# seungjunlee96/lightning-generative-models

Measured on AMD Instinct MI355X. Metric: training images/sec (DDPM UNet 32x32, bs=128), higher is better.
Workload: dtype f32; 1 GPU; configs/diffusion/ddpm.json UNet dim=64, 3x32x32 synthetic NCHW fp32, training_step+backward+Adam+EMA; global_batch=128, per_gpu_batch=128, parallelism=dp1, launch=hipGraph replay (1 graph/step)

## Files before the change

include/lgm_hip.h:

```cpp
#ifndef LGM_HIP_H
#define LGM_HIP_H

#include <stdint.h>

#ifdef __cplusplus
extern "C" {
#endif

#define LGM_ABI_VERSION 7
#define LGM_OK 0
#define LGM_ERR_INVALID (-1)
#define LGM_ERR_UNSUPPORTED (-2)

int lgm_abi_version(void);
const char* lgm_last_error(void);
const char* lgm_last_kernel(void);
int lgm_kernel_name_count(void);
const char* lgm_kernel_name(int i);

typedef struct {
  int32_t B, H, W, Cw;
  int32_t Ho, Wo, Nw;
  int32_t KH, KW, stride, pad;
} LgmConvGeom;
// ... 103 lines not shown
                    const float* g, float* gx, int64_t gx_pitch, int accumulate_gx, const float* res,
                    int64_t res_pitch, float* gg, float gg_beta, int64_t npix, int C, void* workspace, void* stream);
int lgm_rmsnorm_bwd_deferred(const float* x, int64_t x_pitch, const float* gy, int64_t gy_pitch,
                             const float* g, float* gx, int64_t gx_pitch, int accumulate_gx, const float* res,
                             int64_t res_pitch, float* gg, float gg_beta, int64_t npix, int C, void* workspace,
                             int64_t* desc, void* stream);

int lgm_linattn_fwd(const float* qkv, int64_t qkv_pitch, const float* mem_kv, int B, int n,
                    int heads, int dim_head, int M, float* out, int64_t out_pitch, float* ctx,
                    float* kmax, float* ksum, void* stream);
int64_t lgm_rms_qkv_fused_supported(int C, int N);
int lgm_rms_qkv_fused(const float* x, int64_t x_pitch, const float* g, const float* w, int C, int N, int64_t npix,
                      float* xn, int64_t xn_pitch, float* qkv, int64_t qkv_pitch, void* stream);
int64_t lgm_linattn_fwd_fused_supported(int heads, int dim_head, int Cout);
int lgm_linattn_fwd_fused(const float* qkv, int64_t qkv_pitch, const float* mem_kv, int B, int n, int heads,
                          int dim_head, int M, const float* wout, const float* bout, const float* g, int Cout,
                          const float* x, int64_t x_pitch, float* out, int64_t out_pitch, float* o2,
                          int64_t o2_pitch, float* y, int64_t y_pitch, float* ctx, float* kmax, float* ksum,
                          void* stream);
int64_t lgm_linattn_bwd_workspace(int B, int heads, int dim_head, int M);
int lgm_linattn_bwd(const float* qkv, int64_t qkv_pitch, const float* mem_kv, const float* gout,
                    int64_t gout_pitch, const float* ctx, const float* kmax, const float* ksum,
                    int B, int n, int heads, int dim_head, int M, float* gqkv, int64_t gqkv_pitch,
                    float* gmem_kv, float gmem_beta, void* workspace, void* stream);
int64_t lgm_linattn_bwd_fused_supported(int heads, int dim_head, int C);
int64_t lgm_linattn_bwd_fused_slabs(int B, int n, int C);
int64_t lgm_linattn_bwd_fused_workspace(int B, int heads, int dim_head);
int lgm_linattn_bwd_fused(const float* qkv, int64_t qkv_pitch, const float* mem_kv, const float* gout,
                          int64_t gout_pitch, const float* ctx, const float* kmax, const float* ksum,
                          const float* xn, int64_t xn_pitch, const float* wqkv_t, int C, int B, int n,
                          int heads, int dim_head, int M, float* gxn, int64_t gxn_pitch, float* gwqkv,
                          float gw_beta, void* slabs, int64_t slab_bytes, int64_t* gw_desc, float* gmem_kv,
                          float gmem_beta, void* gmem_part, int64_t* gmem_desc, void* workspace, void* stream);
int lgm_linattn_bwd_deferred(const float* qkv, int64_t qkv_pitch, const float* mem_kv, const float* gout,
                             int64_t gout_pitch, const float* ctx, const float* kmax, const float* ksum,
                             int B, int n, int heads, int dim_head, int M, float* gqkv, int64_t gqkv_pitch,
                             float* gmem_kv, float gmem_beta, void* gmem_part, int64_t* gmem_desc,
                             void* workspace, void* stream);
int lgm_attn_bwd_deferred(const float* qkv, int64_t qkv_pitch, const float* mem_kv, const float* out,
                          int64_t out_pitch, const float* gout, int64_t gout_pitch, const float* lse, int B,
                          int n, int heads, int dim_head, int M, float* gqkv, int64_t gqkv_pitch,
                          float* gmem_kv, float gmem_beta, void* gmem_part, int64_t* gmem_desc, void* stream);
int lgm_attn_fwd(const float* qkv, int64_t qkv_pitch, const float* mem_kv, int B, int n, int heads,
                 int dim_head, int M, float* out, int64_t out_pitch, float* lse, void* stream);
int64_t lgm_attn_bwd_workspace(int B, int heads, int dim_head, int M);
int lgm_attn_bwd(const float* qkv, int64_t qkv_pitch, const float* mem_kv, const float* out,
                 int64_t out_pitch, const float* gout, int64_t gout_pitch, const float* lse, int B,
                 int n, int heads, int dim_head, int M, float* gqkv, int64_t gqkv_pitch,
                 float* gmem_kv, float gmem_beta, void* workspace, void* stream);

int lgm_posemb(const int64_t* t, int B, int dim, const float* freqs, float* out, int64_t pitch, void* stream);

#define LGM_ACT_NONE 0
#define LGM_ACT_SILU 1
#define LGM_ACT_GELU 2
#define LGM_ACT_RELU 3
#define LGM_ACT_LRELU 4
#define LGM_ACT_TANH 5
int lgm_act_fwd(const float* x, int64_t x_pitch, const float* bias, const float* res,
                int64_t res_pitch, float* y, int64_t y_pitch, int64_t rows, int cols, int act,
                float slope, void* stream);
int lgm_act_bwd(const float* x, int64_t x_pitch, const float* bias, const float* gy,
                int64_t gy_pitch, float* gx, int64_t gx_pitch, int accumulate, int64_t rows,
                int cols, int act, float slope, void* stream);
int lgm_axpby(const float* a, int64_t a_pitch, float alpha, const float* b, int64_t b_pitch,
              float beta, float* y, int64_t y_pitch, int64_t rows, int cols, void* stream);
// ... 247 lines not shown
```

lightning-generative-models_amd/csrc/attention.hip:

```cpp
#include "lgm_common.h"

int lgm_linattn_ctx_launch(int mode, const float* qkv, long pitch, const float* mem_kv, const float* gout,
                           long gout_pitch, const float* ctx_in, int B, int n, int heads, int M, float scale,
                           float* ctx_out, float* kmax, float* ksum, float* r_out, hipStream_t s,
                           const float* kmax_in = nullptr, const float* ksum_in = nullptr,
                           float* gmem_partial = nullptr);
int lgm_linattn_bwd_fused_launch(const float* qkv, long pitch, const float* gout, long gout_pitch, const float* ctx,
                                 const float* gctx, const float* kmax, const float* ksum, const float* rvec,
                                 const float* xn, long xn_pitch, const float* wt, int B, int n, float scale,
                                 float* gxn, long gxn_pitch, float* slabs, int* blocks_out, hipStream_t s);
int lgm_wgrad_reduce_launch(const float* ws, long slab, float* gw, long n_w, float* gb, long n_b, int splits, float beta,
                            hipStream_t s);
int lgm_linattn_out_fused_launch(const float* qkv, long pitch, const float* ctx, const float* wout, const float* bout,
                                 const float* g, const float* x, long x_pitch, float* ao, long ao_pitch, float* o2,
                                 long o2_pitch, float* y, long y_pitch, int B, int n, int Cout, float scale, hipStream_t s);
int lgm_linattn_bwd_launch(const float* qkv, long pitch, const float* mem_kv, const float* gout, long gout_pitch,
                           const float* ctx, const float* gctx, const float* kmax, const float* ksum,
                           const float* rvec, int B, int n, int heads, int M, float scale, float* gqkv,
                           long gq_pitch, float* gmem_partial, hipStream_t s);
int lgm_attn_tiled_fwd_launch(const float* qkv, long pitch, const float* mem_kv, int B, int n, int heads, int M,
                              float scale, float* out, long out_pitch, float* lse, hipStream_t s);
int lgm_attn_tiled_bwd_launch(const float* qkv, long pitch, const float* mem_kv, const float* out, long out_pitch,
                              const float* gout, long gout_pitch, const float* lse, int B, int n, int heads, int M,
                              float scale, float* gqkv, long gq_pitch, float* gmem_partial, hipStream_t s);

namespace {

constexpr int DH = 32;
constexpr int TI = 64;


__global__ __launch_bounds__(256) void linattn_out_kernel(const float* __restrict__ qkv, long pitch,
                                                          const float* __restrict__ ctx, int n, int heads, float scale,
                                                          float* __restrict__ out, long out_pitch) {
  __shared__ float Qs[TI][DH + 1];
  __shared__ __align__(16) float Cs[DH][DH];
  const int bh = blockIdx.x;
  const int b = bh / heads, h = bh % heads;
  const int i0 = blockIdx.y * TI;
  const int tid = threadIdx.x;
  const int d_l = tid % DH, pl = tid / DH;
  for (int k = tid; k < DH * DH; k += 256) Cs[k / DH][k % DH] = ctx[(long)bh * DH * DH + k];
  {
// ... 488 lines not shown
    gmem_desc[3] = ncols; gmem_desc[4] = 0; gmem_desc[5] = 0; gmem_desc[6] = B; gmem_desc[7] = bb.i;
    return LGM_OK;
  }
  return lgm_wgrad_reduce_launch(part, ncols, gmem_kv, ncols, nullptr, 0, B, gmem_beta, s);
}
}

extern "C" int lgm_linattn_bwd(const float* qkv, int64_t qkv_pitch, const float* mem_kv, const float* gout,
                               int64_t gout_pitch, const float* ctx, const float* kmax, const float* ksum, int B,
                               int n, int heads, int dim_head, int M, float* gqkv, int64_t gqkv_pitch,
                               float* gmem_kv, float gmem_beta, void* workspace, void* stream) {
  LGM_REQUIRE(workspace, "linattn_bwd: null pointer");
  const long bh = (long)B * heads;
  float* part = (float*)workspace + bh * DH * DH + bh * DH;
  return linattn_bwd_impl(qkv, qkv_pitch, mem_kv, gout, gout_pitch, ctx, kmax, ksum, B, n, heads, dim_head, M, gqkv,
                          gqkv_pitch, gmem_kv, gmem_beta, part, nullptr, workspace, stream);
}

extern "C" int lgm_linattn_bwd_deferred(const float* qkv, int64_t qkv_pitch, const float* mem_kv, const float* gout,
                                        int64_t gout_pitch, const float* ctx, const float* kmax, const float* ksum,
                                        int B, int n, int heads, int dim_head, int M, float* gqkv, int64_t gqkv_pitch,
                                        float* gmem_kv, float gmem_beta, void* gmem_part, int64_t* gmem_desc,
                                        void* workspace, void* stream) {
  LGM_REQUIRE(gmem_desc && gmem_part && lgm_aligned16(gmem_kv), "linattn_bwd_deferred: descriptor / partial buffer / aligned gradient required");
  return linattn_bwd_impl(qkv, qkv_pitch, mem_kv, gout, gout_pitch, ctx, kmax, ksum, B, n, heads, dim_head, M, gqkv,
                          gqkv_pitch, gmem_kv, gmem_beta, (float*)gmem_part, gmem_desc, workspace, stream);
}

extern "C" int64_t lgm_linattn_bwd_fused_workspace(int B, int heads, int dim_head) {
  const int64_t bh = (int64_t)B * heads;
  return (bh * dim_head * dim_head + bh * dim_head) * (int64_t)sizeof(float) + 64;
}

extern "C" int lgm_linattn_bwd_fused(const float* qkv, int64_t qkv_pitch, const float* mem_kv, const float* gout,
                                     int64_t gout_pitch, const float* ctx, const float* kmax, const float* ksum,
                                     const float* xn, int64_t xn_pitch, const float* wqkv_t, int C, int B, int n,
                                     int heads, int dim_head, int M, float* gxn, int64_t gxn_pitch, float* gwqkv,
                                     float gw_beta, void* slabs, int64_t slab_bytes, int64_t* gw_desc, float* gmem_kv,
                                     float gmem_beta, void* gmem_part, int64_t* gmem_desc, void* workspace,
                                     void* stream) {
  if (int rc = attn_check(B, n, heads, dim_head, M)) return rc;
  LGM_REQUIRE(lgm_linattn_bwd_fused_supported(heads, dim_head, C), "linattn_bwd_fused: heads=%d dim_head=%d C=%d unsupported",
              heads, dim_head, C);
  LGM_REQUIRE(qkv && mem_kv && gout && ctx && kmax && ksum && xn && wqkv_t && gxn && gwqkv && slabs && gmem_kv && gmem_part &&
                  workspace, "linattn_bwd_fused: null pointer");
  LGM_REQUIRE(qkv_pitch % 4 == 0 && gout_pitch % 4 == 0 && xn_pitch % 4 == 0 && gxn_pitch % 4 == 0 && lgm_aligned16(qkv) &&
                  lgm_aligned16(gout) && lgm_aligned16(ctx) && lgm_aligned16(kmax) && lgm_aligned16(ksum) &&
                  lgm_aligned16(xn) && lgm_aligned16(wqkv_t) && lgm_aligned16(gxn) && lgm_aligned16(gwqkv) &&
                  lgm_aligned16(slabs) && lgm_aligned16(workspace) && lgm_aligned16(gmem_kv) && lgm_aligned16(gmem_part),
              "linattn_bwd_fused: 16-byte aligned operands required");
  LGM_REQUIRE(slab_bytes >= lgm_linattn_bwd_fused_slabs(B, n, C), "linattn_bwd_fused: slab buffer too small");
  hipStream_t s = (hipStream_t)stream;
  const float scale = 1.f / sqrtf((float)dim_head);
  const long bh = (long)B * heads;
  float* gctx = (float*)workspace;
  float* rvec = gctx + bh * DH * DH;
  const long ncols = 2L * heads * DH * M;
  if (int rc = lgm_linattn_ctx_launch(1, qkv, (long)qkv_pitch, mem_kv, gout, (long)gout_pitch, ctx, B, n, heads, M, scale,
                                      gctx, nullptr, nullptr, rvec, s, kmax, ksum, (float*)gmem_part))
    return rc;
  int blocks = 0;
  if (int rc = lgm_linattn_bwd_fused_launch(qkv, (long)qkv_pitch, gout, (long)gout_pitch, ctx, gctx, kmax, ksum, rvec, xn,
                                            (long)xn_pitch, wqkv_t, B, n, scale, gxn, (long)gxn_pitch, (float*)slabs,
                                            &blocks, s))
    return rc;
  union { float f; int64_t i; } bb;
  if (M > 0) {
    if (gmem_desc) {
      bb.i = 0; bb.f = gmem_beta;
      gmem_desc[0] = (int64_t)(uintptr_t)gmem_part; gmem_desc[1] = ncols; gmem_desc[2] = (int64_t)(uintptr_t)gmem_kv;
      gmem_desc[3] = ncols; gmem_desc[4] = 0; gmem_desc[5] = 0; gmem_desc[6] = B; gmem_desc[7] = bb.i;
    } else if (int rc = lgm_wgrad_reduce_launch((const float*)gmem_part, ncols, gmem_kv, ncols, nullptr, 0, B, gmem_beta, s)) {
      return rc;
    }
  } else if (gmem_desc) {
    gmem_desc[6] = 0;
  }
  const long n_w = 3L * heads * DH * C;
  if (gw_desc) {
    bb.i = 0; bb.f = gw_beta;
    gw_desc[0] = (int64_t)(uintptr_t)slabs; gw_desc[1] = n_w; gw_desc[2] = (int64_t)(uintptr_t)gwqkv; gw_desc[3] = n_w;
    gw_desc[4] = 0; gw_desc[5] = 0; gw_desc[6] = blocks; gw_desc[7] = bb.i;
  } else if (int rc = lgm_wgrad_reduce_launch((const float*)slabs, n_w, gwqkv, n_w, nullptr, 0, blocks, gw_beta, s)) {
    return rc;
  }
  return LGM_OK;
}

extern "C" int lgm_attn_fwd(const float* qkv, int64_t qkv_pitch, const float* mem_kv, int B, int n, int heads,
                            int dim_head, int M, float* out, int64_t out_pitch, float* lse, void* stream) {
  if (int rc = attn_check(B, n, heads, dim_head, M)) return rc;
  LGM_REQUIRE(qkv && mem_kv && out && lse, "attn_fwd: null pointer");
  if (attn_tiled(n))
    return lgm_attn_tiled_fwd_launch(qkv, (long)qkv_pitch, mem_kv, B, n, heads, M, 1.f / sqrtf((float)dim_head), out,
                                     (long)out_pitch, lse, (hipStream_t)stream);
  const size_t smem = (size_t)2 * (n + M) * FA_LD * sizeof(float);
  static const bool no_small = getenv("LGM_NO_SMALL_ATTN") != nullptr;
  if (!no_small && n <= SA_MAXN && M <= 16 && qkv_pitch % 4 == 0 && out_pitch % 4 == 0 && lgm_aligned16(qkv) &&
      lgm_aligned16(out) && lgm_aligned16(mem_kv))
  {
    static bool attr = false;
    if (!attr) {
      hipFuncSetAttribute(reinterpret_cast<const void*>(attn_small_fwd_kernel), hipFuncAttributeMaxDynamicSharedMemorySize,
                          (int)(sa_fwd_floats(SA_MAXN, 16) * sizeof(float)));
      attr = true;
    }
    hipLaunchKernelGGL(attn_small_fwd_kernel, dim3(B * heads), dim3(256), sa_fwd_floats(n, M) * sizeof(float),
                       (hipStream_t)stream, qkv, (long)qkv_pitch, mem_kv, n, heads, M, 1.f / sqrtf((float)dim_head), out,
                       (long)out_pitch, lse);
  }
  else
    hipLaunchKernelGGL(attn_fwd_kernel, dim3(B * heads), dim3(128), smem, (hipStream_t)stream, qkv, (long)qkv_pitch,
                       mem_kv, n, heads, M, 1.f / sqrtf((float)dim_head), out, (long)out_pitch, lse);
  LGM_LAUNCH_CHECK();
  return LGM_OK;
}

extern "C" int64_t lgm_attn_bwd_workspace(int B, int heads, int dim_head, int M) {
  const int64_t ncols = 2LL * heads * M * dim_head;
// ... 81 lines not shown
```

lightning-generative-models_amd/csrc/linattn_fused.hip:

```cpp
#include <type_traits>

#include "lgm_common.h"

int lgm_wgrad_reduce_launch(const float* ws, long slab, float* gw, long n_w, float* gb, long n_b, int splits, float beta,
                            hipStream_t s);

namespace {

constexpr int DH = 32;
constexpr int HEADS = 4;
constexpr int HID = HEADS * DH;
constexpr int C = 64;
constexpr int LD = 36;
constexpr int TP = 128;
constexpr int XLD = 80;
constexpr int WLD = 100;

struct FArgs {
  const float* qkv;  long pitch;
  const float* gout; long gout_pitch;
  const float* ctx; const float* gctx; const float* kmax; const float* ksum; const float* rvec;
  const float* xn;   long xn_pitch;
  const float* wt;
  float* gxn;        long gxn_pitch;
  float* slabs;
  int n, tiles, items, per;
  float scale;
};

__device__ __forceinline__ void load16(const float* p, float (&v)[16]) {
#pragma unroll
  for (int q = 0; q < 4; ++q) {
    const f32x4 t = *reinterpret_cast<const f32x4*>(p + 4 * q);
    v[4 * q] = t[0]; v[4 * q + 1] = t[1]; v[4 * q + 2] = t[2]; v[4 * q + 3] = t[3];
  }
}

__global__ __launch_bounds__(256, 1) void linattn_bwd_fused_kernel(const FArgs p) {
  extern __shared__ __align__(16) float sm[];
  float* Qs = sm;
  float* Ks = Qs + TP * LD;
  float* Vs = Ks + TP * LD;
  float* Gs = Vs + TP * LD;
  float* Cs = Gs + TP * LD;
  float* GCs = Cs + DH * LD;
  float* GCt = GCs + DH * LD;
  float* rr = GCt + DH * LD;
  float* Ws = rr + DH;
  float* Xs = Ws + C * WLD;
  const int tid = threadIdx.x;
  const int lane = tid & 63, wid = tid >> 6;
  const int lr = lane & 31, lh = lane >> 5;
  const int l16 = lane & 15, lq = lane >> 4;
  const int c4 = (tid & 7) * 4, prow = tid >> 3;
  const int srow = 32 * wid + (lane >> 1), spart = (lane & 1) * 16;
  const int it0 = blockIdx.x * p.per, it1 = min(p.items, it0 + p.per);
  if (it0 >= it1) return;

  int w_src[6], w_dst[6];
#pragma unroll
  for (int u = 0; u < 6; ++u) {
    const int e = tid + 256 * u;
    const int c = e / 24, rem = e - 24 * c;
    const int part = rem >> 3, j = rem & 7;
    w_src[u] = c * (3 * HID) + part * HID + 4 * j;
    w_dst[u] = c * WLD + part * DH + 4 * j;
  }

  f32x4 q4[4], k4[4], v4[4], g4[4], km4, ks4, cx4, gc4, w4[6];
  float rr1 = 0.f;
  auto issue = [&](int it, int h) {
    const int b = it / p.tiles, i0 = (it % p.tiles) * TP;
    const int rows = min(TP, p.n - i0);
    const long bh = (long)b * HEADS + h;
#pragma unroll
    for (int u = 0; u < 4; ++u) {
      const int r = prow + 32 * u;
      const long row = (long)b * p.n + i0 + (r < rows ? r : 0);
      const float* qp = p.qkv + row * p.pitch + h * DH + c4;
      q4[u] = *reinterpret_cast<const f32x4*>(qp);
      k4[u] = *reinterpret_cast<const f32x4*>(qp + HID);
      v4[u] = *reinterpret_cast<const f32x4*>(qp + 2 * HID);
      g4[u] = *reinterpret_cast<const f32x4*>(p.gout + row * p.gout_pitch + h * DH + c4);
    }
    km4 = *reinterpret_cast<const f32x4*>(p.kmax + bh * DH + c4);
    ks4 = *reinterpret_cast<const f32x4*>(p.ksum + bh * DH + c4);
    cx4 = *reinterpret_cast<const f32x4*>(p.ctx + bh * DH * DH + tid * 4);
    gc4 = *reinterpret_cast<const f32x4*>(p.gctx + bh * DH * DH + tid * 4);
    if (tid < DH) rr1 = p.rvec[bh * DH + tid];
#pragma unroll
    for (int u = 0; u < 6; ++u) w4[u] = *reinterpret_cast<const f32x4*>(p.wt + w_src[u] + h * DH);
  };

  f32x4 dacc[HEADS][6];
#pragma unroll
  for (int h = 0; h < HEADS; ++h)
#pragma unroll
    for (int t = 0; t < 6; ++t) dacc[h][t] = f32x4{0.f, 0.f, 0.f, 0.f};
  const f32x4 zero4 = {0.f, 0.f, 0.f, 0.f};

  issue(it0, 0);
  for (int it = it0; it < it1; ++it) {
    const int b = it / p.tiles, i0 = (it % p.tiles) * TP;
    const int rows = min(TP, p.n - i0);
    f32x16 acc[2];
#pragma unroll
    for (int a = 0; a < 2; ++a)
#pragma unroll
      for (int r = 0; r < 16; ++r) acc[a][r] = 0.f;
    {
#pragma unroll
      for (int u = 0; u < 4; ++u) {
        const int r = prow + 32 * u;
        const long row = (long)b * p.n + i0 + (r < rows ? r : 0);
#pragma unroll
        for (int hf = 0; hf < 2; ++hf) {
          f32x4 xv = *reinterpret_cast<const f32x4*>(p.xn + row * p.xn_pitch + hf * 32 + c4);
          if (r >= rows) xv = zero4;
          *reinterpret_cast<f32x4*>(Xs + r * XLD + hf * 32 + c4) = xv;
        }
      }
    }
    auto head = [&](auto hc) {
      constexpr int h = decltype(hc)::value;
#pragma unroll
      for (int u = 0; u < 4; ++u) {
        const int r = prow + 32 * u;
        const bool live = r < rows;
        f32x4 kv;
#pragma unroll
        for (int k = 0; k < 4; ++k) kv[k] = __expf(k4[u][k] - km4[k]) * (1.f / ks4[k]);
        *reinterpret_cast<f32x4*>(Qs + r * LD + c4) = live ? q4[u] : zero4;
        *reinterpret_cast<f32x4*>(Ks + r * LD + c4) = live ? kv : zero4;
        *reinterpret_cast<f32x4*>(Vs + r * LD + c4) = live ? v4[u] : zero4;
        *reinterpret_cast<f32x4*>(Gs + r * LD + c4) = live ? g4[u] : zero4;
      }
      {
        const int d = tid >> 3, e0 = (tid & 7) * 4;
// ... 70 lines not shown
        dot += __shfl_xor(dot, 1, 64);
#pragma unroll
        for (int q = 0; q < 4; ++q) {
          f32x4 oq, ok;
#pragma unroll
          for (int k = 0; k < 4; ++k) {
            oq[k] = sv[4 * q + k] * (g1[4 * q + k] - dot);
            ok[k] = kk[4 * q + k] * (t2[4 * q + k] - rv[4 * q + k]);
          }
          *reinterpret_cast<f32x4*>(Qs + srow * LD + spart + 4 * q) = oq;
          *reinterpret_cast<f32x4*>(Ks + srow * LD + spart + 4 * q) = ok;
        }
      }
      lgm_wave_lds_sync();
      {
        float* vp = Vs + (32 * wid + lr) * LD + 4 * lh;
#pragma unroll
        for (int g = 0; g < 4; ++g)
          *reinterpret_cast<f32x4*>(vp + 8 * g) = f32x4{a3[4 * g], a3[4 * g + 1], a3[4 * g + 2], a3[4 * g + 3]};
      }
      lgm_wave_lds_sync();
#pragma unroll
      for (int part = 0; part < 3; ++part) {
        float xb[16], w0[16], w1[16];
        load16((part == 0 ? Qs : part == 1 ? Ks : Vs) + (32 * wid + lr) * LD + 16 * lh, xb);
        load16(Ws + lr * WLD + part * DH + 16 * lh, w0);
        load16(Ws + (32 + lr) * WLD + part * DH + 16 * lh, w1);
#pragma unroll
        for (int s = 0; s < 16; ++s) {
          acc[0] = __builtin_amdgcn_mfma_f32_32x32x2f32(w0[s], xb[s], acc[0], 0, 0, 0);
          acc[1] = __builtin_amdgcn_mfma_f32_32x32x2f32(w1[s], xb[s], acc[1], 0, 0, 0);
        }
      }
      __syncthreads();
      {
        const float* xb = Xs + lq * XLD + 16 * wid + l16;
#pragma unroll 4
        for (int s = 0; s < TP / 4; ++s) {
          const float bv = xb[4 * s * XLD];
#pragma unroll
          for (int part = 0; part < 3; ++part) {
            const float* X = (part == 0 ? Qs : part == 1 ? Ks : Vs) + (4 * s + lq) * LD + l16;
            dacc[h][2 * part] = __builtin_amdgcn_mfma_f32_16x16x4f32(X[0], bv, dacc[h][2 * part], 0, 0, 0);
            dacc[h][2 * part + 1] = __builtin_amdgcn_mfma_f32_16x16x4f32(X[16], bv, dacc[h][2 * part + 1], 0, 0, 0);
          }
        }
        __syncthreads();
      }
    };
    head(std::integral_constant<int, 0>{});
    head(std::integral_constant<int, 1>{});
    head(std::integral_constant<int, 2>{});
    head(std::integral_constant<int, 3>{});
    if (32 * wid + lr < rows) {
      float* o = p.gxn + ((long)b * p.n + i0 + 32 * wid + lr) * p.gxn_pitch + 4 * lh;
#pragma unroll
      for (int a = 0; a < 2; ++a)
#pragma unroll
        for (int g = 0; g < 4; ++g)
          *reinterpret_cast<f32x4*>(o + 32 * a + 8 * g) = f32x4{acc[a][4 * g], acc[a][4 * g + 1], acc[a][4 * g + 2], acc[a][4 * g + 3]};
    }
  }
  {
    float* sl = p.slabs + (long)blockIdx.x * (3 * HID * C);
#pragma unroll
    for (int h = 0; h < HEADS; ++h)
#pragma unroll
      for (int t = 0; t < 6; ++t)
#pragma unroll
        for (int r = 0; r < 4; ++r) {
          const int wrow = (t >> 1) * HID + h * DH + (t & 1) * 16 + 4 * lq + r;
          sl[(long)wrow * C + 16 * wid + l16] = dacc[h][t][r];
        }
  }
}

constexpr size_t kSmem = ((size_t)4 * TP * LD + 3 * DH * LD + DH + C * WLD + TP * XLD) * sizeof(float);

int plan_blocks(int B, int n, int* tiles, int* items, int* per) {
  *tiles = lgm_cdiv(n, TP);
  *items = B * *tiles;
  const int nb = *items < 256 ? *items : 256;
  *per = lgm_cdiv(*items, nb);
  return lgm_cdiv(*items, *per);
}

}

extern "C" int64_t lgm_linattn_bwd_fused_supported(int heads, int dim_head, int Cin) {
  return heads == HEADS && dim_head == DH && Cin == C ? 1 : 0;
}

extern "C" int64_t lgm_linattn_bwd_fused_slabs(int B, int n, int Cin) {
  if (Cin != C) return 0;
  int tiles, items, per;
  const int blocks = plan_blocks(B, n, &tiles, &items, &per);
  return (int64_t)blocks * 3 * HID * C * (int64_t)sizeof(float);
}

int lgm_linattn_bwd_fused_launch(const float* qkv, long pitch, const float* gout, long gout_pitch, const float* ctx,
                                 const float* gctx, const float* kmax, const float* ksum, const float* rvec,
                                 const float* xn, long xn_pitch, const float* wt, int B, int n, float scale,
                                 float* gxn, long gxn_pitch, float* slabs, int* blocks_out, hipStream_t s) {
  FArgs a;
  a.qkv = qkv; a.pitch = pitch; a.gout = gout; a.gout_pitch = gout_pitch;
  a.ctx = ctx; a.gctx = gctx; a.kmax = kmax; a.ksum = ksum; a.rvec = rvec;
  a.xn = xn; a.xn_pitch = xn_pitch; a.wt = wt; a.gxn = gxn; a.gxn_pitch = gxn_pitch;
  a.slabs = slabs; a.n = n; a.scale = scale;
  const int blocks = plan_blocks(B, n, &a.tiles, &a.items, &a.per);
  *blocks_out = blocks;
  lgm_note_kernel(LGM_KNAME("linattn_bwd_fused_kernel"));
  static bool attr = false;
  if (!attr) {
    (void)hipFuncSetAttribute(reinterpret_cast<const void*>(linattn_bwd_fused_kernel),
                              hipFuncAttributeMaxDynamicSharedMemorySize, (int)kSmem);
    attr = true;
  }
  hipLaunchKernelGGL(linattn_bwd_fused_kernel, dim3(blocks), dim3(256), kSmem, s, a);
  LGM_LAUNCH_CHECK();
  return LGM_OK;
}

namespace {

constexpr int OTP = 128;
constexpr int ALD = 132;

struct OArgs {
  const float* qkv;  long pitch;
  const float* ctx;
  const float* wout; const float* bout; const float* g;
  const float* x;    long x_pitch;
  float* ao;         long ao_pitch;
  float* o2;         long o2_pitch;
  float* y;          long y_pitch;
  int n, tiles, items, per;
  float scale;
};

template <int NC>
__global__ __launch_bounds__(256, NC == 2 ? 3 : 1) void linattn_out_fused_kernel(const OArgs p) {
  constexpr int CO = 32 * NC;
  extern __shared__ __align__(16) float sm[];
  float* Ws = sm;
  float* Ct = Ws + CO * ALD;
  const int tid = threadIdx.x;
  const int lane = tid & 63, wid = tid >> 6;
  const int lr = lane & 31, lh = lane >> 5;
  const int it0 = blockIdx.x * p.per, it1 = min(p.items, it0 + p.per);
  if (it0 >= it1) return;
  const float sqrtc = sqrtf((float)CO);
// ... 311 lines not shown
```

lightning-generative-models_amd/lgm_hip/ops.py:

```python
from __future__ import annotations

import ctypes
from typing import Optional

import torch

from ._lib import ConvGeom, lib

ACT_NONE, ACT_SILU, ACT_GELU, ACT_RELU, ACT_LRELU, ACT_TANH = 0, 1, 2, 3, 4, 5


def stream() -> int:
    return torch.cuda.current_stream().cuda_stream


def _p(t: Optional[torch.Tensor]) -> Optional[int]:
    return None if t is None else t.data_ptr()


def pitch(t: torch.Tensor) -> int:
    assert t.stride(-1) == 1 or t.shape[-1] == 1, "last dim must be dense"
    if t.dim() == 1:
        return t.shape[0]
    pt = t.stride(-2)
# ... 962 lines not shown
    L = lib()
    B, H, W, _ = qkv.shape
    ws = workspace(L.lgm_linattn_bwd_workspace(B, heads, dim_head, M), qkv.device)
    if defer is None or gmem_ptr % 16 or M <= 0:
        L.lgm_linattn_bwd(qkv.data_ptr(), pitch(qkv), mem_ptr, gout.data_ptr(), pitch(gout), ctx.data_ptr(),
                          kstat[0].data_ptr(), kstat[1].data_ptr(), B, H * W, heads, dim_head, M, gqkv.data_ptr(),
                          pitch(gqkv), gmem_ptr, gmem_beta, ws.data_ptr(), stream())
        return
    nb = B * 2 * heads * dim_head * M * 4
    part = _persistent((gmem_ptr, nb), nb, qkv.device)
    desc = (ctypes.c_int64 * 8)()
    L.lgm_linattn_bwd_deferred(qkv.data_ptr(), pitch(qkv), mem_ptr, gout.data_ptr(), pitch(gout), ctx.data_ptr(),
                               kstat[0].data_ptr(), kstat[1].data_ptr(), B, H * W, heads, dim_head, M, gqkv.data_ptr(),
                               pitch(gqkv), gmem_ptr, gmem_beta, part.data_ptr(), ctypes.addressof(desc), ws.data_ptr(),
                               stream())
    if desc[6] > 0:
        defer.append(tuple(desc))


LA_FUSED = _os.environ.get("LGM_NO_LA_FUSED") is None
LA_FUSED_MIN_ITEMS = int(_os.environ.get("LGM_LA_FUSED_MIN_ITEMS", "256"))


def linattn_bwd_fused_ok(heads, dim_head, C, qkv, gout, xn, wt_ptr, gw_ptr, gmem_ptr) -> bool:
    if not LA_FUSED or not wt_ptr or not lib().lgm_linattn_bwd_fused_supported(heads, dim_head, C):
        return False
    B, H, W, _ = qkv.shape
    if B * ((H * W + 127) // 128) < LA_FUSED_MIN_ITEMS:
        return False
    return not any(v % 16 for v in (qkv.data_ptr(), gout.data_ptr(), xn.data_ptr(), wt_ptr, gw_ptr, gmem_ptr)) and \
        pitch(qkv) % 4 == 0 and pitch(gout) % 4 == 0 and pitch(xn) % 4 == 0


def linattn_bwd_fused(qkv, mem_ptr, gout, ctx, kstat, xn, wt_ptr, heads, dim_head, M, gxn, gw_ptr, gw_beta, gw_defer,
                      gmem_ptr, gmem_beta, gmem_defer):
    L = lib()
    B, H, W, _ = qkv.shape
    n, C = H * W, xn.shape[-1]
    dev = qkv.device
    wsb = L.lgm_linattn_bwd_fused_workspace(B, heads, dim_head)
    slab_bytes = L.lgm_linattn_bwd_fused_slabs(B, n, C)
    part_bytes = B * 2 * heads * dim_head * M * 4
    extra = (0 if gw_defer is not None else slab_bytes + 64) + (0 if gmem_defer is not None else part_bytes + 64)
    ws = workspace(wsb + extra + 64, dev)
    off = (wsb + 63) // 64 * 64
    if gmem_defer is not None:
        part_ptr = _persistent((gmem_ptr, part_bytes), part_bytes, dev).data_ptr()
    else:
        part_ptr = ws.data_ptr() + off
        off += (part_bytes + 63) // 64 * 64
    slab_ptr = _persistent((gw_ptr, slab_bytes), slab_bytes, dev).data_ptr() if gw_defer is not None \
        else ws.data_ptr() + off
    d_w = (ctypes.c_int64 * 8)() if gw_defer is not None else None
    d_m = (ctypes.c_int64 * 8)() if gmem_defer is not None else None
    L.lgm_linattn_bwd_fused(qkv.data_ptr(), pitch(qkv), mem_ptr, gout.data_ptr(), pitch(gout), ctx.data_ptr(),
                            kstat[0].data_ptr(), kstat[1].data_ptr(), xn.data_ptr(), pitch(xn), wt_ptr, C, B, n, heads,
                            dim_head, M, gxn.data_ptr(), pitch(gxn), gw_ptr, gw_beta, slab_ptr, slab_bytes,
                            None if d_w is None else ctypes.addressof(d_w), gmem_ptr, gmem_beta, part_ptr,
                            None if d_m is None else ctypes.addressof(d_m), ws.data_ptr(), stream())
    if d_w is not None and d_w[6] > 0:
        gw_defer.append(tuple(d_w))
    if d_m is not None and d_m[6] > 0:
        gmem_defer.append(tuple(d_m))


def attn_fwd(qkv, mem_ptr, heads, dim_head, M, out):
    B, H, W, _ = qkv.shape
    lse = new((B, heads, H * W), qkv)
    lib().lgm_attn_fwd(qkv.data_ptr(), pitch(qkv), mem_ptr, B, H * W, heads, dim_head, M, out.data_ptr(),
                       pitch(out), lse.data_ptr(), stream())
    return lse


def attn_bwd(qkv, mem_ptr, out, gout, lse, heads, dim_head, M, gqkv, gmem_ptr, gmem_beta, defer=None):
    L = lib()
    B, H, W, _ = qkv.shape
    if defer is None or gmem_ptr % 16 or M <= 0:
        ws = workspace(L.lgm_attn_bwd_workspace(B, heads, dim_head, M), qkv.device)
        L.lgm_attn_bwd(qkv.data_ptr(), pitch(qkv), mem_ptr, out.data_ptr(), pitch(out), gout.data_ptr(),
                       pitch(gout), lse.data_ptr(), B, H * W, heads, dim_head, M, gqkv.data_ptr(), pitch(gqkv),
                       gmem_ptr, gmem_beta, ws.data_ptr(), stream())
        return
    nb = B * 2 * heads * dim_head * M * 4
    part = _persistent((gmem_ptr, nb), nb, qkv.device)
    desc = (ctypes.c_int64 * 8)()
    L.lgm_attn_bwd_deferred(qkv.data_ptr(), pitch(qkv), mem_ptr, out.data_ptr(), pitch(out), gout.data_ptr(),
                            pitch(gout), lse.data_ptr(), B, H * W, heads, dim_head, M, gqkv.data_ptr(), pitch(gqkv),
                            gmem_ptr, gmem_beta, part.data_ptr(), ctypes.addressof(desc), stream())
    if desc[6] > 0:
        defer.append(tuple(desc))


_POSEMB_FREQS = {}


def posemb_freqs(dim, theta, device) -> torch.Tensor:
# ... 116 lines not shown
```

lightning-generative-models_amd/models/generative/diffusion/ddpm.py:

```python
from __future__ import annotations

import math
import os
from collections import namedtuple
from typing import List, Optional, Tuple

import torch
from torch import nn

from lgm_hip import ops
from lgm_hip.flat import FlatParams, _r4
from lgm_hip.lightning import LightningModule, multi_rank
from lgm_hip.nn import Conv2d, GradCtx, GroupNorm, Linear, RMSNorm, param_kind
from lgm_hip.optim import EMA, FusedAdam


ModelPrediction = namedtuple("ModelPrediction", ["pred_noise", "pred_x_start"])


_NO_RES_FOLD = os.environ.get("LGM_NO_RES_FOLD") is not None


def _chan(t: torch.Tensor, lo: int, hi: int) -> torch.Tensor:
    return t[..., lo:hi]
# ... 63 lines not shown
        B, H, W, C = x.shape
        fp = self.mem_kv._lgm_flat
        r = ops.rms_qkv_fused(x, fp.ptr(self.norm.g), fp.ptr(self.to_qkv.weight), 3 * self.heads * self.dim_head)
        if r is not None:
            xn, qkv = r
        else:
            xn = self.norm.fwd(x)
            qkv = self.to_qkv.fwd(xn)
        ao = ops.new((B, H, W, self.heads * self.dim_head), x)
        conv, norm = self.to_out[0], self.to_out[1]
        if ops.linattn_fwd_fused_ok(self.heads, self.dim_head, C, qkv, x, fp.ptr(conv.weight), fp.ptr(conv.bias),
                                    fp.ptr(norm.g)) and out.data_ptr() % 16 == 0 and ops.pitch(out) % 4 == 0:
            o2 = ops.new((B, H, W, C), x)
            ctx, kstat = ops.linattn_fwd_fused(qkv, fp.ptr(self.mem_kv), self.heads, self.dim_head, self.M,
                                               fp.ptr(conv.weight), fp.ptr(conv.bias), fp.ptr(norm.g), x, ao, o2, out)
        else:
            ctx, kstat = ops.linattn_fwd(qkv, fp.ptr(self.mem_kv), self.heads, self.dim_head, self.M, ao)
            o2 = conv.fwd(ao)
            norm.fwd(o2, res=x, out=out)
        return (x, xn, qkv, ao, ctx, kstat, o2) if save else None

    def bwd(self, gc: GradCtx, saved, gy, gx, accumulate: bool):
        x, xn, qkv, ao, ctx, kstat, o2 = saved
        fp = gc.flat
        go2 = self.to_out[1].bwd(gc, o2, gy)
        gao = self.to_out[0].bwd(gc, ao, go2)
        del go2
        w = self.to_qkv.weight
        gqkv = None
        if ops.linattn_bwd_fused_ok(self.heads, self.dim_head, xn.shape[-1], qkv, gao, xn, fp.tptr(w), fp.gptr(w),
                                    fp.gptr(self.mem_kv)):
            dw, dm = gc.defer_for(w), gc.defer_for(self.mem_kv)
            bw, bm = gc.beta(w), gc.beta(self.mem_kv)
            gxn = ops.new(xn.shape, xn)
            ops.linattn_bwd_fused(qkv, fp.ptr(self.mem_kv), gao, ctx, kstat, xn, fp.tptr(w), self.heads, self.dim_head,
                                  self.M, gxn, fp.gptr(w), bw, dw, fp.gptr(self.mem_kv), bm, dm)
        else:
            gqkv = ops.new(qkv.shape, qkv)
            dm = gc.defer_for(self.mem_kv)
            ops.linattn_bwd(qkv, fp.ptr(self.mem_kv), gao, ctx, kstat, self.heads, self.dim_head, self.M, gqkv,
                            fp.gptr(self.mem_kv), gc.beta(self.mem_kv), defer=dm)
            gxn = self.to_qkv.bwd(gc, xn, gqkv)
        del gqkv, gao
        self.norm.bwd(gc, x, gxn, gx, accumulate, res=gy)
        return gx


class Attention(nn.Module):

    def __init__(self, dim, heads=4, dim_head=32, num_mem_kv=4, flash=False):
        super().__init__()
        self.heads, self.dim_head, self.M = heads, dim_head, num_mem_kv
        hidden = heads * dim_head
        self.norm = RMSNorm(dim)
        self.mem_kv = nn.Parameter(torch.randn(2, heads, num_mem_kv, dim_head))
        self.to_qkv = Conv2d(dim, hidden * 3, 1, bias=False)
        self.to_out = Conv2d(hidden, dim, 1)

    def fwd(self, x, out, save: bool):
        B, H, W, C = x.shape
        fp = self.mem_kv._lgm_flat
        r = ops.rms_qkv_fused(x, fp.ptr(self.norm.g), fp.ptr(self.to_qkv.weight), 3 * self.heads * self.dim_head)
        if r is not None:
            xn, qkv = r
        else:
            xn = self.norm.fwd(x)
# ... 842 lines not shown
```

Before: 13610 images/s.

## Fuse RMSNorm backward into fused linear-attention backward kernel epilogue

Adds an RMS variant of the fused linear-attention backward kernel. Its epilogue computes the RMSNorm input gradient, adds the residual gradient, and writes per-block partial sums for the norm gain gradient. These partials are reduced later, either by a deferred descriptor or by a wgrad reduce launch. This removes the separate gxn intermediate buffer and the standalone RMSNorm backward kernel. In exchange it adds register pressure and extra loads inside the kernel, plus an LDS column reduction and an extra __syncthreads per tile.

```diff
diff --git a/include/lgm_hip.h b/include/lgm_hip.h
--- a/include/lgm_hip.h
+++ b/include/lgm_hip.h
@@ -159,6 +159,15 @@
                           int heads, int dim_head, int M, float* gxn, int64_t gxn_pitch, float* gwqkv,
                           float gw_beta, void* slabs, int64_t slab_bytes, int64_t* gw_desc, float* gmem_kv,
                           float gmem_beta, void* gmem_part, int64_t* gmem_desc, void* workspace, void* stream);
+int64_t lgm_linattn_bwd_fused_rms_slabs(int B, int n, int C);
+int lgm_linattn_bwd_fused_rms(const float* qkv, int64_t qkv_pitch, const float* mem_kv, const float* gout,
+                              int64_t gout_pitch, const float* ctx, const float* kmax, const float* ksum,
+                              const float* xn, int64_t xn_pitch, const float* wqkv_t, int C, int B, int n,
+                              int heads, int dim_head, int M, const float* x, int64_t x_pitch, const float* g,
+                              const float* res, int64_t res_pitch, float* gx, int64_t gx_pitch, int accumulate_gx,
+                              float* gg, float gg_beta, int64_t* gg_desc, float* gwqkv, float gw_beta, void* slabs,
+                              int64_t slab_bytes, int64_t* gw_desc, float* gmem_kv, float gmem_beta, void* gmem_part,
+                              int64_t* gmem_desc, void* workspace, void* stream);
 int lgm_linattn_bwd_deferred(const float* qkv, int64_t qkv_pitch, const float* mem_kv, const float* gout,
                              int64_t gout_pitch, const float* ctx, const float* kmax, const float* ksum,
                              int B, int n, int heads, int dim_head, int M, float* gqkv, int64_t gqkv_pitch,
diff --git a/lightning-generative-models_amd/csrc/attention.hip b/lightning-generative-models_amd/csrc/attention.hip
--- a/lightning-generative-models_amd/csrc/attention.hip
+++ b/lightning-generative-models_amd/csrc/attention.hip
@@ -8,7 +8,10 @@
 int lgm_linattn_bwd_fused_launch(const float* qkv, long pitch, const float* gout, long gout_pitch, const float* ctx,
                                  const float* gctx, const float* kmax, const float* ksum, const float* rvec,
                                  const float* xn, long xn_pitch, const float* wt, int B, int n, float scale,
-                                 float* gxn, long gxn_pitch, float* slabs, int* blocks_out, hipStream_t s);
+                                 float* gxn, long gxn_pitch, float* slabs, int* blocks_out, hipStream_t s,
+                                 const float* x = nullptr, long x_pitch = 0, const float* g = nullptr,
+                                 const float* res = nullptr, long res_pitch = 0, float* gx = nullptr, long gx_pitch = 0,
+                                 int accumulate = 0, float* gg_rows = nullptr);
 int lgm_wgrad_reduce_launch(const float* ws, long slab, float* gw, long n_w, float* gb, long n_b, int splits, float beta,
                             hipStream_t s);
 int lgm_linattn_out_fused_launch(const float* qkv, long pitch, const float* ctx, const float* wout, const float* bout,
@@ -563,24 +566,38 @@
   return (bh * dim_head * dim_head + bh * dim_head) * (int64_t)sizeof(float) + 64;
 }
 
-extern "C" int lgm_linattn_bwd_fused(const float* qkv, int64_t qkv_pitch, const float* mem_kv, const float* gout,
-                                     int64_t gout_pitch, const float* ctx, const float* kmax, const float* ksum,
-                                     const float* xn, int64_t xn_pitch, const float* wqkv_t, int C, int B, int n,
-                                     int heads, int dim_head, int M, float* gxn, int64_t gxn_pitch, float* gwqkv,
-                                     float gw_beta, void* slabs, int64_t slab_bytes, int64_t* gw_desc, float* gmem_kv,
-                                     float gmem_beta, void* gmem_part, int64_t* gmem_desc, void* workspace,
-                                     void* stream) {
+namespace {
+struct LaRms {
+  const float* x; int64_t x_pitch; const float* g; const float* res; int64_t res_pitch;
+  float* gx; int64_t gx_pitch; int accumulate; float* gg; float gg_beta; int64_t* gg_desc;
+};
+
+int linattn_bwd_fused_impl(const float* qkv, int64_t qkv_pitch, const float* mem_kv, const float* gout,
+                           int64_t gout_pitch, const float* ctx, const float* kmax, const float* ksum,
+                           const float* xn, int64_t xn_pitch, const float* wqkv_t, int C, int B, int n,
+                           int heads, int dim_head, int M, float* gxn, int64_t gxn_pitch, float* gwqkv,
+                           float gw_beta, void* slabs, int64_t slab_bytes, int64_t* gw_desc, float* gmem_kv,
+                           float gmem_beta, void* gmem_part, int64_t* gmem_desc, void* workspace, void* stream,
+                           const LaRms* rms) {
   if (int rc = attn_check(B, n, heads, dim_head, M)) return rc;
   LGM_REQUIRE(lgm_linattn_bwd_fused_supported(heads, dim_head, C), "linattn_bwd_fused: heads=%d dim_head=%d C=%d unsupported",
               heads, dim_head, C);
-  LGM_REQUIRE(qkv && mem_kv && gout && ctx && kmax && ksum && xn && wqkv_t && gxn && gwqkv && slabs && gmem_kv && gmem_part &&
-                  workspace, "linattn_bwd_fused: null pointer");
+  LGM_REQUIRE(qkv && mem_kv && gout && ctx && kmax && ksum && xn && wqkv_t && (gxn || rms) && gwqkv && slabs && gmem_kv &&
+                  gmem_part && workspace, "linattn_bwd_fused: null pointer");
   LGM_REQUIRE(qkv_pitch % 4 == 0 && gout_pitch % 4 == 0 && xn_pitch % 4 == 0 && gxn_pitch % 4 == 0 && lgm_aligned16(qkv) &&
                   lgm_aligned16(gout) && lgm_aligned16(ctx) && lgm_aligned16(kmax) && lgm_aligned16(ksum) &&
                   lgm_aligned16(xn) && lgm_aligned16(wqkv_t) && lgm_aligned16(gxn) && lgm_aligned16(gwqkv) &&
                   lgm_aligned16(slabs) && lgm_aligned16(workspace) && lgm_aligned16(gmem_kv) && lgm_aligned16(gmem_part),
               "linattn_bwd_fused: 16-byte aligned operands required");
-  LGM_REQUIRE(slab_bytes >= lgm_linattn_bwd_fused_slabs(B, n, C), "linattn_bwd_fused: slab buffer too small");
+  if (rms) {
+    LGM_REQUIRE(rms->x && rms->g && rms->res && rms->gx && rms->gg, "linattn_bwd_fused_rms: null pointer");
+    LGM_REQUIRE(rms->x_pitch % 4 == 0 && rms->res_pitch % 4 == 0 && rms->gx_pitch % 4 == 0 && lgm_aligned16(rms->x) &&
+                    lgm_aligned16(rms->g) && lgm_aligned16(rms->res) && lgm_aligned16(rms->gx) && lgm_aligned16(rms->gg),
+                "linattn_bwd_fused_rms: 16-byte aligned operands required");
+    LGM_REQUIRE(slab_bytes >= lgm_linattn_bwd_fused_rms_slabs(B, n, C), "linattn_bwd_fused_rms: slab buffer too small");
+  } else {
+    LGM_REQUIRE(slab_bytes >= lgm_linattn_bwd_fused_slabs(B, n, C), "linattn_bwd_fused: slab buffer too small");
+  }
   hipStream_t s = (hipStream_t)stream;
   const float scale = 1.f / sqrtf((float)dim_head);
   const long bh = (long)B * heads;
@@ -591,10 +608,16 @@
                                       gctx, nullptr, nullptr, rvec, s, kmax, ksum, (float*)gmem_part))
     return rc;
   int blocks = 0;
-  if (int rc = lgm_linattn_bwd_fused_launch(qkv, (long)qkv_pitch, gout, (long)gout_pitch, ctx, gctx, kmax, ksum, rvec, xn,
-                                            (long)xn_pitch, wqkv_t, B, n, scale, gxn, (long)gxn_pitch, (float*)slabs,
-                                            &blocks, s))
-    return rc;
+  const long n_w = 3L * heads * DH * C;
+  int rc = rms ? lgm_linattn_bwd_fused_launch(qkv, (long)qkv_pitch, gout, (long)gout_pitch, ctx, gctx, kmax, ksum, rvec,
+                                              xn, (long)xn_pitch, wqkv_t, B, n, scale, nullptr, 0, (float*)slabs, &blocks,
+                                              s, rms->x, (long)rms->x_pitch, rms->g, rms->res, (long)rms->res_pitch,
+                                              rms->gx, (long)rms->gx_pitch, rms->accumulate,
+                                              (float*)slabs + (long)lgm_linattn_bwd_fused_slabs(B, n, C) / 4)
+               : lgm_linattn_bwd_fused_launch(qkv, (long)qkv_pitch, gout, (long)gout_pitch, ctx, gctx, kmax, ksum, rvec,
+                                              xn, (long)xn_pitch, wqkv_t, B, n, scale, gxn, (long)gxn_pitch, (float*)slabs,
+                                              &blocks, s);
+  if (rc) return rc;
   union { float f; int64_t i; } bb;
   if (M > 0) {
     if (gmem_desc) {
@@ -607,7 +630,6 @@
   } else if (gmem_desc) {
     gmem_desc[6] = 0;
   }
-  const long n_w = 3L * heads * DH * C;
   if (gw_desc) {
     bb.i = 0; bb.f = gw_beta;
     gw_desc[0] = (int64_t)(uintptr_t)slabs; gw_desc[1] = n_w; gw_desc[2] = (int64_t)(uintptr_t)gwqkv; gw_desc[3] = n_w;
@@ -615,7 +637,46 @@
   } else if (int rc = lgm_wgrad_reduce_launch((const float*)slabs, n_w, gwqkv, n_w, nullptr, 0, blocks, gw_beta, s)) {
     return rc;
   }
+  if (rms) {
+    const float* rows = (const float*)slabs + (long)blocks * n_w;
+    if (rms->gg_desc) {
+      bb.i = 0; bb.f = rms->gg_beta;
+      int64_t* d = rms->gg_desc;
+      d[0] = (int64_t)(uintptr_t)rows; d[1] = C; d[2] = (int64_t)(uintptr_t)rms->gg; d[3] = C;
+      d[4] = 0; d[5] = 0; d[6] = blocks; d[7] = bb.i;
+    } else if (int rc = lgm_wgrad_reduce_launch(rows, C, rms->gg, C, nullptr, 0, blocks, rms->gg_beta, s)) {
+      return rc;
+    }
+  }
   return LGM_OK;
+}
+}
+
+extern "C" int lgm_linattn_bwd_fused(const float* qkv, int64_t qkv_pitch, const float* mem_kv, const float* gout,
+                                     int64_t gout_pitch, const float* ctx, const float* kmax, const float* ksum,
+                                     const float* xn, int64_t xn_pitch, const float* wqkv_t, int C, int B, int n,
+                                     int heads, int dim_head, int M, float* gxn, int64_t gxn_pitch, float* gwqkv,
+                                     float gw_beta, void* slabs, int64_t slab_bytes, int64_t* gw_desc, float* gmem_kv,
+                                     float gmem_beta, void* gmem_part, int64_t* gmem_desc, void* workspace,
+                                     void* stream) {
+  return linattn_bwd_fused_impl(qkv, qkv_pitch, mem_kv, gout, gout_pitch, ctx, kmax, ksum, xn, xn_pitch, wqkv_t, C, B, n,
+                                heads, dim_head, M, gxn, gxn_pitch, gwqkv, gw_beta, slabs, slab_bytes, gw_desc, gmem_kv,
+                                gmem_beta, gmem_part, gmem_desc, workspace, stream, nullptr);
+}
+
+extern "C" int lgm_linattn_bwd_fused_rms(const float* qkv, int64_t qkv_pitch, const float* mem_kv, const float* gout,
+                                         int64_t gout_pitch, const float* ctx, const float* kmax, const float* ksum,
+                                         const float* xn, int64_t xn_pitch, const float* wqkv_t, int C, int B, int n,
+                                         int heads, int dim_head, int M, const float* x, int64_t x_pitch, const float* g,
+                                         const float* res, int64_t res_pitch, float* gx, int64_t gx_pitch,
+                                         int accumulate_gx, float* gg, float gg_beta, int64_t* gg_desc, float* gwqkv,
+                                         float gw_beta, void* slabs, int64_t slab_bytes, int64_t* gw_desc,
+                                         float* gmem_kv, float gmem_beta, void* gmem_part, int64_t* gmem_desc,
+                                         void* workspace, void* stream) {
+  const LaRms rms{x, x_pitch, g, res, res_pitch, gx, gx_pitch, accumulate_gx, gg, gg_beta, gg_desc};
+  return linattn_bwd_fused_impl(qkv, qkv_pitch, mem_kv, gout, gout_pitch, ctx, kmax, ksum, xn, xn_pitch, wqkv_t, C, B, n,
+                                heads, dim_head, M, nullptr, 0, gwqkv, gw_beta, slabs, slab_bytes, gw_desc, gmem_kv,
+                                gmem_beta, gmem_part, gmem_desc, workspace, stream, &rms);
 }
 
 extern "C" int lgm_attn_fwd(const float* qkv, int64_t qkv_pitch, const float* mem_kv, int B, int n, int heads,
diff --git a/lightning-generative-models_amd/csrc/linattn_fused.hip b/lightning-generative-models_amd/csrc/linattn_fused.hip
--- a/lightning-generative-models_amd/csrc/linattn_fused.hip
+++ b/lightning-generative-models_amd/csrc/linattn_fused.hip
@@ -26,6 +26,12 @@
   float* slabs;
   int n, tiles, items, per;
   float scale;
+  const float* x;    long x_pitch;
+  const float* g;
+  const float* res;  long res_pitch;
+  float* gx;         long gx_pitch;
+  float* gg_rows;
+  int accumulate;
 };
 
 __device__ __forceinline__ void load16(const float* p, float (&v)[16]) {
@@ -36,6 +42,7 @@
   }
 }
 
+template <bool RMS>
 __global__ __launch_bounds__(256, 1) void linattn_bwd_fused_kernel(const FArgs p) {
   extern __shared__ __align__(16) float sm[];
   float* Qs = sm;
@@ -99,11 +106,14 @@
     for (int t = 0; t < 6; ++t) dacc[h][t] = f32x4{0.f, 0.f, 0.f, 0.f};
   const f32x4 zero4 = {0.f, 0.f, 0.f, 0.f};
 
+  float ggw = 0.f;
+
   issue(it0, 0);
   for (int it = it0; it < it1; ++it) {
     const int b = it / p.tiles, i0 = (it % p.tiles) * TP;
     const int rows = min(TP, p.n - i0);
     f32x16 acc[2];
+    f32x4 ex[RMS ? 8 : 1];
 #pragma unroll
     for (int a = 0; a < 2; ++a)
 #pragma unroll
@@ -240,6 +250,14 @@
           acc[1] = __builtin_amdgcn_mfma_f32_32x32x2f32(w1[s], xb[s], acc[1], 0, 0, 0);
         }
       }
+      if constexpr (RMS && h == HEADS - 1) {
+        const long row = (long)b * p.n + i0 + min(32 * wid + lr, rows - 1);
+#pragma unroll
+        for (int a = 0; a < 2; ++a)
+#pragma unroll
+          for (int g = 0; g < 4; ++g)
+            ex[4 * a + g] = *reinterpret_cast<const f32x4*>(p.x + row * p.x_pitch + 32 * a + 8 * g + 4 * lh);
+      }
       __syncthreads();
       {
         const float* xb = Xs + lq * XLD + 16 * wid + l16;
@@ -260,7 +278,62 @@
     head(std::integral_constant<int, 1>{});
     head(std::integral_constant<int, 2>{});
     head(std::integral_constant<int, 3>{});
-    if (32 * wid + lr < rows) {
+    if constexpr (RMS) {
+      const int r = 32 * wid + lr;
+      const bool live = r < rows;
+      const long row = (long)b * p.n + i0 + min(r, rows - 1);
+      const float sqrtc = sqrtf((float)C);
+      float ss = 0.f;
+#pragma unroll
+      for (int k = 0; k < 8; ++k) ss += ex[k][0] * ex[k][0] + ex[k][1] * ex[k][1] + ex[k][2] * ex[k][2] + ex[k][3] * ex[k][3];
+      ss += __shfl_xor(ss, 32, 64);
+      const float nrm = sqrtf(ss);
+      const bool clamped = nrm < 1e-12f;
+      const float invn = 1.f / fmaxf(nrm, 1e-12f);
+      float* red = Qs + (64 * wid + lane) * LD;
+      auto xh_gxh = [&](int a, int g, f32x4& xh, f32x4& gxh, f32x4& gi) {
+        gi = f32x4{acc[a][4 * g], acc[a][4 * g + 1], acc[a][4 * g + 2], acc[a][4 * g + 3]};
+        const f32x4 gv = *reinterpret_cast<const f32x4*>(p.g + 32 * a + 8 * g + 4 * lh);
+        xh = ex[4 * a + g] * invn;
+        gxh = gi * gv * sqrtc;
+      };
+      float dot = 0.f;
+#pragma unroll
+      for (int a = 0; a < 2; ++a)
+#pragma unroll
+        for (int g = 0; g < 4; ++g) {
+          f32x4 xh, gxh, gi;
+          xh_gxh(a, g, xh, gxh, gi);
+          *reinterpret_cast<f32x4*>(red + 4 * (4 * a + g)) = live ? gi * xh * sqrtc : zero4;
+          dot += xh[0] * gxh[0] + xh[1] * gxh[1] + xh[2] * gxh[2] + xh[3] * gxh[3];
+        }
+      dot += __shfl_xor(dot, 32, 64);
+      if (clamped) dot = 0.f;
+      if (live) {
+#pragma unroll
+        for (int a = 0; a < 2; ++a)
+#pragma unroll
+          for (int g = 0; g < 4; ++g) {
+            f32x4 xh, gxh, gi;
+            xh_gxh(a, g, xh, gxh, gi);
+            f32x4 o = (gxh - xh * dot) * invn;
+            float* dst = p.gx + row * p.gx_pitch + 32 * a + 8 * g + 4 * lh;
+            if (p.accumulate) o += *reinterpret_cast<const f32x4*>(dst);
+            o += *reinterpret_cast<const f32x4*>(p.res + row * p.res_pitch + 32 * a + 8 * g + 4 * lh);
+            *reinterpret_cast<f32x4*>(dst) = o;
+          }
+      }
+      lgm_wave_lds_sync();
+      {
+        const int k = 4 * (4 * (lane >> 5) + ((lane >> 3) & 3)) + (lane & 3);
+        const float* col = Qs + (64 * wid + 32 * ((lane >> 2) & 1)) * LD + k;
+        float s = 0.f;
+#pragma unroll 8
+        for (int l = 0; l < 32; ++l) s += col[l * LD];
+        ggw += s;
+      }
+      __syncthreads();
+    } else if (32 * wid + lr < rows) {
       float* o = p.gxn + ((long)b * p.n + i0 + 32 * wid + lr) * p.gxn_pitch + 4 * lh;
 #pragma unroll
       for (int a = 0; a < 2; ++a)
@@ -280,6 +353,12 @@
           const int wrow = (t >> 1) * HID + h * DH + (t & 1) * 16 + 4 * lq + r;
           sl[(long)wrow * C + 16 * wid + l16] = dacc[h][t][r];
         }
+  }
+  if constexpr (RMS) {
+    __syncthreads();
+    sm[tid] = ggw;
+    __syncthreads();
+    if (tid < C) p.gg_rows[(long)blockIdx.x * C + tid] = ((sm[tid] + sm[64 + tid]) + sm[128 + tid]) + sm[192 + tid];
   }
 }
 
@@ -306,25 +385,47 @@
   return (int64_t)blocks * 3 * HID * C * (int64_t)sizeof(float);
 }
 
+extern "C" int64_t lgm_linattn_bwd_fused_rms_slabs(int B, int n, int Cin) {
+  if (Cin != C) return 0;
+  int tiles, items, per;
+  const int blocks = plan_blocks(B, n, &tiles, &items, &per);
+  return (int64_t)blocks * (3 * HID * C + C) * (int64_t)sizeof(float);
+}
+
 int lgm_linattn_bwd_fused_launch(const float* qkv, long pitch, const float* gout, long gout_pitch, const float* ctx,
                                  const float* gctx, const float* kmax, const float* ksum, const float* rvec,
                                  const float* xn, long xn_pitch, const float* wt, int B, int n, float scale,
-                                 float* gxn, long gxn_pitch, float* slabs, int* blocks_out, hipStream_t s) {
+                                 float* gxn, long gxn_pitch, float* slabs, int* blocks_out, hipStream_t s,
+                                 const float* x, long x_pitch, const float* g, const float* res, long res_pitch,
+                                 float* gx, long gx_pitch, int accumulate, float* gg_rows) {
   FArgs a;
   a.qkv = qkv; a.pitch = pitch; a.gout = gout; a.gout_pitch = gout_pitch;
   a.ctx = ctx; a.gctx = gctx; a.kmax = kmax; a.ksum = ksum; a.rvec = rvec;
   a.xn = xn; a.xn_pitch = xn_pitch; a.wt = wt; a.gxn = gxn; a.gxn_pitch = gxn_pitch;
   a.slabs = slabs; a.n = n; a.scale = scale;
+  a.x = x; a.x_pitch = x_pitch; a.g = g; a.res = res; a.res_pitch = res_pitch; a.gx = gx; a.gx_pitch = gx_pitch;
+  a.gg_rows = gg_rows; a.accumulate = accumulate;
   const int blocks = plan_blocks(B, n, &a.tiles, &a.items, &a.per);
   *blocks_out = blocks;
-  lgm_note_kernel(LGM_KNAME("linattn_bwd_fused_kernel"));
-  static bool attr = false;
-  if (!attr) {
-    (void)hipFuncSetAttribute(reinterpret_cast<const void*>(linattn_bwd_fused_kernel),
-                              hipFuncAttributeMaxDynamicSharedMemorySize, (int)kSmem);
-    attr = true;
-  }
-  hipLaunchKernelGGL(linattn_bwd_fused_kernel, dim3(blocks), dim3(256), kSmem, s, a);
+  if (gx) {
+    lgm_note_kernel(LGM_KNAME("linattn_bwd_fused_kernel<true>"));
+    static bool attr = false;
+    if (!attr) {
+      (void)hipFuncSetAttribute(reinterpret_cast<const void*>(linattn_bwd_fused_kernel<true>),
+                                hipFuncAttributeMaxDynamicSharedMemorySize, (int)kSmem);
+      attr = true;
+    }
+    hipLaunchKernelGGL(linattn_bwd_fused_kernel<true>, dim3(blocks), dim3(256), kSmem, s, a);
+  } else {
+    lgm_note_kernel(LGM_KNAME("linattn_bwd_fused_kernel<false>"));
+    static bool attr = false;
+    if (!attr) {
+      (void)hipFuncSetAttribute(reinterpret_cast<const void*>(linattn_bwd_fused_kernel<false>),
+                                hipFuncAttributeMaxDynamicSharedMemorySize, (int)kSmem);
+      attr = true;
+    }
+    hipLaunchKernelGGL(linattn_bwd_fused_kernel<false>, dim3(blocks), dim3(256), kSmem, s, a);
+  }
   LGM_LAUNCH_CHECK();
   return LGM_OK;
 }
diff --git a/lightning-generative-models_amd/lgm_hip/ops.py b/lightning-generative-models_amd/lgm_hip/ops.py
--- a/lightning-generative-models_amd/lgm_hip/ops.py
+++ b/lightning-generative-models_amd/lgm_hip/ops.py
@@ -1018,16 +1018,28 @@
         pitch(qkv) % 4 == 0 and pitch(gout) % 4 == 0 and pitch(xn) % 4 == 0
 
 
+LA_BWD_RMS = _os.environ.get("LGM_NO_LA_BWD_RMS") is None
+
+
+def linattn_bwd_fused_rms_ok(x, g_ptr, res, gx, gg_ptr) -> bool:
+    if not LA_BWD_RMS:
+        return False
+    return not any(v % 16 for v in (x.data_ptr(), g_ptr, res.data_ptr(), gx.data_ptr(), gg_ptr)) and \
+        pitch(x) % 4 == 0 and pitch(res) % 4 == 0 and pitch(gx) % 4 == 0
+
+
 def linattn_bwd_fused(qkv, mem_ptr, gout, ctx, kstat, xn, wt_ptr, heads, dim_head, M, gxn, gw_ptr, gw_beta, gw_defer,
-                      gmem_ptr, gmem_beta, gmem_defer):
+                      gmem_ptr, gmem_beta, gmem_defer, rms=None):
     L = lib()
     B, H, W, _ = qkv.shape
     n, C = H * W, xn.shape[-1]
     dev = qkv.device
     wsb = L.lgm_linattn_bwd_fused_workspace(B, heads, dim_head)
-    slab_bytes = L.lgm_linattn_bwd_fused_slabs(B, n, C)
+    slab_bytes = L.lgm_linattn_bwd_fused_rms_slabs(B, n, C) if rms is not None else L.lgm_linattn_bwd_fused_slabs(B, n, C)
+    gg_defer = rms[7] if rms is not None else None
+    slab_kept = gw_defer is not None or gg_defer is not None
     part_bytes = B * 2 * heads * dim_head * M * 4
-    extra = (0 if gw_defer is not None else slab_bytes + 64) + (0 if gmem_defer is not None else part_bytes + 64)
+    extra = (0 if slab_kept else slab_bytes + 64) + (0 if gmem_defer is not None else part_bytes + 64)
     ws = workspace(wsb + extra + 64, dev)
     off = (wsb + 63) // 64 * 64
     if gmem_defer is not None:
@@ -1035,19 +1047,31 @@
     else:
         part_ptr = ws.data_ptr() + off
         off += (part_bytes + 63) // 64 * 64
-    slab_ptr = _persistent((gw_ptr, slab_bytes), slab_bytes, dev).data_ptr() if gw_defer is not None \
-        else ws.data_ptr() + off
+    slab_ptr = _persistent((gw_ptr, slab_bytes), slab_bytes, dev).data_ptr() if slab_kept else ws.data_ptr() + off
     d_w = (ctypes.c_int64 * 8)() if gw_defer is not None else None
     d_m = (ctypes.c_int64 * 8)() if gmem_defer is not None else None
-    L.lgm_linattn_bwd_fused(qkv.data_ptr(), pitch(qkv), mem_ptr, gout.data_ptr(), pitch(gout), ctx.data_ptr(),
-                            kstat[0].data_ptr(), kstat[1].data_ptr(), xn.data_ptr(), pitch(xn), wt_ptr, C, B, n, heads,
-                            dim_head, M, gxn.data_ptr(), pitch(gxn), gw_ptr, gw_beta, slab_ptr, slab_bytes,
-                            None if d_w is None else ctypes.addressof(d_w), gmem_ptr, gmem_beta, part_ptr,
-                            None if d_m is None else ctypes.addressof(d_m), ws.data_ptr(), stream())
+    d_g = (ctypes.c_int64 * 8)() if gg_defer is not None else None
+    if rms is None:
+        L.lgm_linattn_bwd_fused(qkv.data_ptr(), pitch(qkv), mem_ptr, gout.data_ptr(), pitch(gout), ctx.data_ptr(),
+                                kstat[0].data_ptr(), kstat[1].data_ptr(), xn.data_ptr(), pitch(xn), wt_ptr, C, B, n,
+                                heads, dim_head, M, gxn.data_ptr(), pitch(gxn), gw_ptr, gw_beta, slab_ptr, slab_bytes,
+                                None if d_w is None else ctypes.addressof(d_w), gmem_ptr, gmem_beta, part_ptr,
+                                None if d_m is None else ctypes.addressof(d_m), ws.data_ptr(), stream())
+    else:
+        x, g_ptr, res, gx, accumulate, gg_ptr, gg_beta, _ = rms
+        L.lgm_linattn_bwd_fused_rms(qkv.data_ptr(), pitch(qkv), mem_ptr, gout.data_ptr(), pitch(gout), ctx.data_ptr(),
+                                    kstat[0].data_ptr(), kstat[1].data_ptr(), xn.data_ptr(), pitch(xn), wt_ptr, C, B, n,
+                                    heads, dim_head, M, x.data_ptr(), pitch(x), g_ptr, res.data_ptr(), pitch(res),
+                                    gx.data_ptr(), pitch(gx), 1 if accumulate else 0, gg_ptr, gg_beta,
+                                    None if d_g is None else ctypes.addressof(d_g), gw_ptr, gw_beta, slab_ptr,
+                                    slab_bytes, None if d_w is None else ctypes.addressof(d_w), gmem_ptr, gmem_beta,
+                                    part_ptr, None if d_m is None else ctypes.addressof(d_m), ws.data_ptr(), stream())
     if d_w is not None and d_w[6] > 0:
         gw_defer.append(tuple(d_w))
     if d_m is not None and d_m[6] > 0:
         gmem_defer.append(tuple(d_m))
+    if d_g is not None and d_g[6] > 0:
+        gg_defer.append(tuple(d_g))
 
 
 def attn_fwd(qkv, mem_ptr, heads, dim_head, M, out):
diff --git a/lightning-generative-models_amd/models/generative/diffusion/ddpm.py b/lightning-generative-models_amd/models/generative/diffusion/ddpm.py
--- a/lightning-generative-models_amd/models/generative/diffusion/ddpm.py
+++ b/lightning-generative-models_amd/models/generative/diffusion/ddpm.py
@@ -119,6 +119,13 @@
                                     fp.gptr(self.mem_kv)):
             dw, dm = gc.defer_for(w), gc.defer_for(self.mem_kv)
             bw, bm = gc.beta(w), gc.beta(self.mem_kv)
+            g = self.norm.g
+            if gx is not None and ops.linattn_bwd_fused_rms_ok(x, fp.ptr(g), gy, gx, fp.gptr(g)):
+                dg = gc.defer_for(g)
+                ops.linattn_bwd_fused(qkv, fp.ptr(self.mem_kv), gao, ctx, kstat, xn, fp.tptr(w), self.heads,
+                                      self.dim_head, self.M, None, fp.gptr(w), bw, dw, fp.gptr(self.mem_kv), bm, dm,
+                                      rms=(x, fp.ptr(g), gy, gx, accumulate, fp.gptr(g), gc.beta(g), dg))
+                return gx
             gxn = ops.new(xn.shape, xn)
             ops.linattn_bwd_fused(qkv, fp.ptr(self.mem_kv), gao, ctx, kstat, xn, fp.tptr(w), self.heads, self.dim_head,
                                   self.M, gxn, fp.gptr(w), bw, dw, fp.gptr(self.mem_kv), bm, dm)
```

Result: no change. 13650 images/s, median of 6 (+0.3%).
